# zaiisao/ConTEXTure-NeRF

Hardware: AMD Instinct MI355X
Metric: UNet denoise steps/sec (CFG-batched SD2-depth UNet eval + PLMS update) (higher is better)
Workload: dtype f16; 1 GPU; BASELINE configs[1]: 1 view @768^2 (latent 96^2), 50 PLMS steps (51 UNet evals), SD2-depth UNet fp16, CFG batch 2, guidance 10, random-init weights; mesh substitution napoleon.obj -> n/a for this stage (denoise loop only); latent=96, cfg_batch=2, ctx_len=77, views_per_rank=1, parallelism=view-shard x1

## Files before the change

### contexture-nerf_amd/_lib.py

```python
import ctypes as C
import os
import torch

_HERE = os.path.dirname(os.path.abspath(__file__))
LIB_PATH = os.path.join(_HERE, "libctxnerf.so")

_vp, _i32, _i64, _f32 = C.c_void_p, C.c_int32, C.c_int64, C.c_float

SIGNATURES = {
    "ctx_version": (_i32, []),
    "ctx_last_error": (C.c_char_p, []),
    "ctx_device_check": (_i32, []),
    "ctx_prepare_vertices": (_i32, [_vp, _vp, _vp, _vp, _i32, _i32, _i32, _vp, _vp, _vp, _vp, _vp]),
    "ctx_rasterize_ws_bytes": (_i64, [_i32, _i32, _i32, _i32]),
    "ctx_rasterize_fwd": (_i32, [_i32, _i32, _vp, _vp, _vp, _i32, _i32, _i32, _f32, _f32, _vp, _vp, _vp, _i64, _vp]),
    "ctx_rasterize_fused": (_i32, [_i32, _i32, _vp, _vp, _vp, _i32, _vp, _i32, _i32, _f32, _f32, _vp, _vp, _vp, _vp, _vp, _i64, _vp]),
    "ctx_normalize_depth_ws_bytes": (_i64, [_i32]),
    "ctx_normalize_depth": (_i32, [_vp, _i32, _i32, _vp, _vp, _vp, _vp]),
    "ctx_texture_mapping_fwd": (_i32, [_vp, _vp, _i32, _i32, _i32, _i32, _i32, _i32, _vp, _vp, _vp]),
    "ctx_texture_mapping_bwd": (_i32, [_vp, _vp, _i32, _i32, _i32, _i32, _vp, _vp, _vp]),
    "ctx_texmap_bwd_plan_bytes": (_i64, [_i32, _i32, _i32]),
    "ctx_texmap_bwd_plan": (_i32, [_vp, _vp, _i32, _i32, _i32, _vp, _vp]),
    "ctx_texture_mapping_bwd_binned_ws_bytes": (_i64, [_i32, _i32]),
    "ctx_texture_mapping_bwd_binned": (_i32, [_vp, _vp, _vp, _i32, _i32, _i32, _i32, _vp, _vp, _vp, _vp]),
# ... 109 lines not shown
    "ctx_vae_encode": (_i32, [_vp, _vp, _i32, _i32, _i32, _vp, _vp]),
    "ctx_vae_flops": (C.c_double, [_vp]),
    "ctx_vae_encode_train_workspace_bytes": (_i64, [_vp, _i32, _i32, _i32]),
    "ctx_vae_encode_train": (_i32, [_vp, _vp, _i32, _i32, _i32, _vp, _vp]),
    "ctx_vae_encode_bwd": (_i32, [_vp, _vp, _f32, _vp, _vp]),
    "ctx_gemm_f16": (_i32, [_vp, _vp, _vp, _vp, _i32, _i32, _i32, _vp, _vp]),
    "ctx_conv3x3_f16": (_i32, [_vp, _vp, _vp, _vp, _vp, _i32, _i32, _i32, _i32, _i32, _i32, _i32, _vp, _vp]),
    "ctx_conv3x3_seg_f16": (_i32, [_vp, _vp, _vp, _vp, _vp, _vp, _i32, _i32, _i32, _i32, _i32, _vp, _vp, _i32, _i32, _vp, _vp, _i32, _i32,
                                   _vp, _i32, _vp, _vp]),
    "ctx_conv3x3_gn_f16": (_i32, [_vp, _vp, _vp, _vp, _vp, _vp, _i32, _i32, _i32, _i32, _i32, _vp, _i32, _i32, _i32, _vp, _vp, _vp, _vp]),
    "ctx_gemm_last_kernel": (None, [_vp, _vp]),
    "ctx_conv3x3_geom_f16": (_i32, [_vp, _vp, _vp, _vp, _i32, _i32, _i32, _i32, _i32, _i32, _i32, _i32, _i32, _vp, _i32, _vp, _vp]),
    "ctx_pack_conv3_dgrad_f16": (_i32, [_vp, _i32, _i32, _i32, _vp, _vp]),
    "ctx_pack_conv3_phase_f16": (_i32, [_vp, _i32, _i32, _vp, _vp]),
    "ctx_conv3x3_phase_f16": (_i32, [_vp, _vp, _vp, _vp, _vp, _i32, _i32, _i32, _i32, _i32, _vp, _i32, _vp, _vp]),
    "ctx_pack_mat_dgrad_f16": (_i32, [_vp, _i32, _i32, _i32, _i32, _vp, _vp]),
    "ctx_groupnorm_bwd_ws_bytes": (_i64, [_i32, _i32]),
    "ctx_groupnorm_bwd_f16": (_i32, [_vp, _vp, _vp, _vp, _vp, _i32, _i32, _i32, _i32, _f32, _i32, _vp, _vp, _vp]),
    "ctx_softmax_rows_f16": (_i32, [_vp, _i32, _i32, _f32, _vp, _vp]),
    "ctx_softmax_bwd_rows_f16": (_i32, [_vp, _vp, _i32, _i32, _f32, _vp, _vp]),
    "ctx_quant_bwd_f16": (_i32, [_vp, _vp, _i32, _i32, _i64, _f32, _vp, _vp]),
    "ctx_conv_in_bwd_f16": (_i32, [_vp, _vp, _i32, _i32, _i32, _i32, _i32, _f32, _vp, _vp]),
    "ctx_conv_in_f16": (_i32, [_vp, _vp, _vp, _i32, _i32, _i32, _i32, _i32, _vp, _vp]),
    "ctx_conv_out_f16": (_i32, [_vp, _vp, _vp, _i32, _i32, _i32, _i32, _i32, _vp, _vp]),
    "ctx_gemv_f16": (_i32, [_vp, _vp, _vp, _i32, _i32, _i32, _i32, _i32, _vp, _vp]),
    "ctx_time_embed_f16": (_i32, [_vp, _i32, _i32, _vp, _vp]),
    "ctx_transpose_v_f16": (_i32, [_vp, _i32, _i32, _i32, _i32, _i32, _vp, _vp]),
    "ctx_concat_f16": (_i32, [_vp, _vp, _i64, _i32, _i32, _vp, _vp]),
    "ctx_concat_f32": (_i32, [_vp, _vp, _i64, _i32, _i32, _vp, _vp]),
    "ctx_f32_to_f16": (_i32, [_vp, _i64, _vp, _vp]),
    "ctx_f16_to_f32": (_i32, [_vp, _i64, _vp, _vp]),
    "ctx_conv_small_f16": (_i32, [_vp, _vp, _vp, _vp, _i32, _i32, _i32, _i32, _i32, _i32, _i32, _vp, _vp]),
    "ctx_add_scaled_f16": (_i32, [_vp, _vp, _f32, _i64, _vp]),
    "ctx_pointwise_f32": (_i32, [_vp, _vp, _vp, _i32, _i32, _i64, _i32, _vp, _vp]),
    "ctx_pack_fwd_f16": (_i32, [_vp, _i32, _i32, _i32, _vp, _vp]),
    "ctx_groupnorm_f16": (_i32, [_vp, _vp, _vp, _i32, _i32, _i32, _i32, _f32, _i32, _vp, _vp, _vp]),
    "ctx_groupnorm2_f16": (_i32, [_vp, _vp, _i32, _vp, _vp, _i32, _i32, _i32, _i32, _f32, _i32, _vp, _vp, _vp]),
    "ctx_groupnorm_apply_f16": (_i32, [_vp, _vp, _i32, _vp, _vp, _i32, _i32, _i32, _i32, _f32, _i32, _vp, _vp]),
    "ctx_groupnorm_slabs_f16": (_i32, [_vp, _i32, _vp, _vp, _vp, _i32, _vp, _vp, _i32, _i32, _i32, _i32, _f32, _i32, _vp, _vp]),
    "ctx_layernorm_f16": (_i32, [_vp, _vp, _vp, _i64, _i32, _f32, _vp, _vp]),
    "ctx_attention_ws_bytes": (_i64, [_i32, _i32, _i32]),
    "ctx_attention_f16": (_i32, [_vp, _vp, _vp, _i32, _i32, _i32, _i32, _i32, _i32, _f32, _vp, _i32, _vp, _vp]),
    "ctx_groupnorm_ws_bytes": (_i64, [_i32, _i32]),
    "ctx_geglu_f16": (_i32, [_vp, _i64, _i32, _vp, _vp]),
    "ctx_profile_begin": (_i32, []),
    "ctx_profile_end": (_i32, [_i32, _vp, _vp]),
# ... 61 lines not shown
```

### contexture-nerf_amd/csrc/elementwise.hip

```cpp
#include "common.h"
#include "kernels.h"
#include <math.h>

__global__ __launch_bounds__(256) void k_geglu(const f16 *__restrict__ h, int64_t M, int C4, f16 *__restrict__ y)
{
    const int c8n = C4 / 8;
    const int64_t total = M * c8n;
    for (int64_t i = (int64_t)blockIdx.x * 256 + threadIdx.x; i < total; i += (int64_t)gridDim.x * 256) {
        int64_t m = i / c8n;
        int c8 = (int)(i % c8n);
        f16x8 a = *(const f16x8 *)(h + m * 2 * C4 + c8 * 8);
        f16x8 g = *(const f16x8 *)(h + m * 2 * C4 + C4 + c8 * 8);
        f16x8 o;
#pragma unroll
        for (int j = 0; j < 8; ++j) {
            float gf = (float)g[j];
            o[j] = (f16)((float)a[j] * (0.5f * gf * (1.0f + erff(gf * 0.70710678118654752f))));
        }
        *(f16x8 *)(y + m * C4 + c8 * 8) = o;
    }
}

extern "C" int32_t ctx_geglu_f16(const void *h, int64_t M, int32_t C4, void *y, ctx_stream_t stream)
{
// ... 88 lines not shown
}

__global__ void k_time_embed(const float *__restrict__ t, int B, int dim, f16 *__restrict__ out)
{
    int i = blockIdx.x * blockDim.x + threadIdx.x;
    int half = dim / 2;
    if (i >= half) return;
    float fr = expf(-9.210340371976184f * (float)i / (float)half);
    float a = t[0] * fr;
    float c = cosf(a), sn = sinf(a);
    for (int b = 0; b < B; ++b) {
        out[(size_t)b * dim + i] = (f16)c;
        out[(size_t)b * dim + half + i] = (f16)sn;
    }
}
int ctx_time_embed_core(const float *t, int B, int dim, f16 *out, hipStream_t s)
{
    CTX_REQUIRE(t && out && B > 0 && dim >= 2 && dim % 2 == 0, "time_embed: unsupported B=%d dim=%d", B, dim);
    hipLaunchKernelGGL(k_time_embed, dim3(cdiv(dim / 2, 64)), dim3(64), 0, s, t, B, dim, out);
    CTX_CHECK_LAUNCH("time_embed");
    return CTX_OK;
}

#define CI_SPLIT 16
template <int CP, int CX>
__global__ __launch_bounds__(256) void k_conv_in(const float *__restrict__ x, const f16 *__restrict__ w,
                                                 const f16 *__restrict__ bias, int B, int Cin, int H, int W, int Cout,
                                                 f16 *__restrict__ y)
{
    extern __shared__ __attribute__((aligned(16))) float s_w[];
    constexpr int WR = 9 * CP, WX = 9 * CX;
    const int o8n = Cout / 8;
    const int o8_per = (o8n + CI_SPLIT - 1) / CI_SPLIT;
    const int o8_0 = blockIdx.y * o8_per, o8_1 = min(o8n, o8_0 + o8_per);
    const int no = (o8_1 - o8_0) * 8;
    for (int i = threadIdx.x; i < no * WX; i += 256) {
        const int o = i / WX, r = i - o * WX, t = r / CX, c = r - t * CX;
        s_w[i] = (float)w[(size_t)(o8_0 * 8 + o) * WR + t * CP + c];
    }
    __syncthreads();
    const int64_t npix = (int64_t)B * H * W;
    const int64_t pix0 = (int64_t)blockIdx.x * 256;
    const int64_t pix = pix0 + threadIdx.x;
    const bool live = pix < npix;
    const int64_t pq = live ? pix : npix - 1;
    int b = (int)(pq / (H * W)), p = (int)(pq % (H * W));
    int oy = p / W, ox = p % W;
    float in[9][CX];
#pragma unroll
    for (int t = 0; t < 9; ++t) {
        int iy = oy + t / 3 - 1, ix = ox + t % 3 - 1;
        bool ok = iy >= 0 && iy < H && ix >= 0 && ix < W;
#pragma unroll
        for (int c = 0; c < CX; ++c)
            in[t][c] = (ok && c < Cin) ? (float)(f16)x[(((size_t)b * Cin + c) * H + iy) * W + ix] : 0.f;
    }
    f16 *patch = (f16 *)(s_w + no * WX);
    for (int g0 = o8_0; g0 < o8_1; g0 += 8) {
        const int ng = min(8, o8_1 - g0);
        for (int gi = 0; gi < ng; ++gi) {
            const int o8 = g0 + gi;
            f16x8 o;
#pragma unroll
            for (int j = 0; j < 8; ++j) {
                const float *wr = s_w + ((o8 - o8_0) * 8 + j) * WX;
                float acc = (float)bias[o8 * 8 + j];
#pragma unroll
                for (int t = 0; t < 9; ++t)
#pragma unroll
                    for (int c = 0; c < CX; ++c) acc += in[t][c] * wr[t * CX + c];
                o[j] = (f16)acc;
            }
            *(f16x8 *)(patch + threadIdx.x * 72 + gi * 8) = o;
        }
        __syncthreads();
        for (int ch = threadIdx.x; ch < 256 * ng; ch += 256) {
            const int px = ch / ng, gi = ch - px * ng;
            if (pix0 + px < npix) *(f16x8 *)(y + (pix0 + px) * Cout + (g0 + gi) * 8) = *(const f16x8 *)(patch + px * 72 + gi * 8);
        }
        __syncthreads();
    }
}
int ctx_conv_in_core(const float *x, const f16 *w, const f16 *bias, int B, int Cin, int H, int W, int Cout, f16 *y, hipStream_t s)
{
    CTX_REQUIRE(x && w && bias && y && Cout > 0 && Cout % 8 == 0, "conv_in: unsupported Cout=%d", Cout);
    CTX_REQUIRE(Cin >= 1 && Cin <= 16, "conv_in: need 1 <= Cin <= 16 (Cin=%d)", Cin);
    CTX_REQUIRE(B > 0 && H > 0 && W > 0 && (int64_t)H * W < (1ll << 31), "conv_in: unsupported grid B=%d H=%d W=%d", B, H, W);
    int64_t npix = (int64_t)B * H * W;
    int o8_per = (Cout / 8 + CI_SPLIT - 1) / CI_SPLIT;
    const int cx = Cin <= 3 ? 3 : Cin <= 5 ? Cin : Cin <= 8 ? 8 : Cin == 9 ? 9 : 16;
    CTX_REQUIRE((size_t)o8_per * 8 * 9 * cx * sizeof(float) + 256 * 72 * sizeof(f16) <= 64 * 1024,
                "conv_in: the weight slice of Cout=%d at Cin=%d does not fit the LDS", Cout, Cin);
    const dim3 grid((unsigned)cdiv64(npix, 256), CI_SPLIT);
#define CI_GO(CP_, CX_) hipLaunchKernelGGL((k_conv_in<CP_, CX_>), grid, dim3(256), (size_t)o8_per * 8 * 9 * CX_ * sizeof(float) + 256 * 72 * sizeof(f16), s, x, w, bias, B, Cin, H, W, Cout, y)
    if (Cin <= 3) CI_GO(8, 3);
    else if (Cin == 4) CI_GO(8, 4);
    else if (Cin == 5) CI_GO(8, 5);
    else if (Cin <= 8) CI_GO(8, 8);
    else if (Cin == 9) CI_GO(16, 9);
    else CI_GO(16, 16);
#undef CI_GO
    CTX_CHECK_LAUNCH("conv_in");
    return CTX_OK;
}

template <int NU, bool WF32>
__global__ __launch_bounds__(256) void k_conv_out(const f16 *__restrict__ x, const f16 *__restrict__ w,
                                                  const f16 *__restrict__ bias, int B, int H, int W, int C, int Cout,
                                                  float *__restrict__ out)
{
    extern __shared__ __attribute__((aligned(16))) char s_cw_raw[];
    f16 *s_cw = (f16 *)s_cw_raw;
    float *s_cf = (float *)s_cw_raw;
    const int nwt = Cout * 9 * C;
    if (WF32) {
        for (int i = threadIdx.x * 8; i < nwt; i += 256 * 8) {
            const f16x8 v = *(const f16x8 *)(w + i);
#pragma unroll
            for (int j = 0; j < 8; ++j) s_cf[i + j] = (float)v[j];
        }
    } else {
        for (int i = threadIdx.x * 8; i < nwt; i += 256 * 8) *(f16x8 *)(s_cw + i) = *(const f16x8 *)(w + i);
    }
// ... 135 lines not shown
}
extern "C" int32_t ctx_transpose_v_f16(const void *v, int32_t B, int32_t S, int32_t ld, int32_t heads, int32_t Sp, void *vt, ctx_stream_t stream)
{
    CTX_REQUIRE(B <= 65535 && heads <= 65535, "transpose_v: B=%d / heads=%d exceed the grid", B, heads);
    return ctx_transpose_v_core((const f16 *)v, B, S, ld, heads, Sp, (f16 *)vt, (hipStream_t)stream);
}
extern "C" int32_t ctx_f32_to_f16(const float *x, int64_t n, void *y, ctx_stream_t stream)
{
    return ctx_f32_to_f16_core(x, n, (f16 *)y, (hipStream_t)stream);
}
extern "C" int32_t ctx_f16_to_f32(const void *x, int64_t n, float *y, ctx_stream_t stream)
{
    return ctx_f16_to_f32_core((const f16 *)x, n, y, (hipStream_t)stream);
}
extern "C" int32_t ctx_time_embed_f16(const float *t, int32_t B, int32_t dim, void *out, ctx_stream_t stream)
{
    return ctx_time_embed_core(t, B, dim, (f16 *)out, (hipStream_t)stream);
}
extern "C" int32_t ctx_conv_in_f16(const float *x, const void *w_pack, const void *bias, int32_t B, int32_t Cin, int32_t H, int32_t W, int32_t Cout,
                                   void *y, ctx_stream_t stream)
{
    return ctx_conv_in_core(x, (const f16 *)w_pack, (const f16 *)bias, B, Cin, H, W, Cout, (f16 *)y, (hipStream_t)stream);
}
extern "C" int32_t ctx_conv_out_f16(const void *x, const void *w, const void *bias, int32_t B, int32_t H, int32_t W, int32_t C, int32_t Cout,
                                    float *out, ctx_stream_t stream)
{
    return ctx_conv_out_core((const f16 *)x, (const f16 *)w, (const f16 *)bias, B, H, W, C, Cout, out, (hipStream_t)stream);
}
```

### contexture-nerf_amd/csrc/gemm.hip

```cpp
#include "gemm_common.h"

template <int MI, int NI, bool PH = false>
__device__ __forceinline__ void gemm_epilogue(const GemmArgs &a, f32x16 (&acc)[MI][NI], int mw, int nw, int r, int h, const ConvPhase &ph)
{
#pragma unroll
    for (int mi = 0; mi < MI; ++mi) {
        int m = mw + mi * 32 + r;
        if (m >= ph.M) continue;
        const int mo = PH ? conv_phase_row(a, ph, m) : m;
        int bidx = a.rowbias ? m / a.rows_per_batch : 0;
        if (a.epi == 1) {
            if constexpr (NI == 2) {
                int fbase = nw / 2;
#pragma unroll
                for (int g = 0; g < 4; ++g) {
                    int nn = nw + 8 * g + 4 * h;
                    if (nn >= a.N) continue;
                    f16x4 o;
#pragma unroll
                    for (int j = 0; j < 4; ++j) {
                        float xv = acc[mi][0][4 * g + j], gv = acc[mi][1][4 * g + j];
                        if (a.bias) { xv += (float)a.bias[nn + j]; gv += (float)a.bias[nn + 32 + j]; }
                        o[j] = geglu(xv, gv);
                    }
// ... 666 lines not shown
                                      int32_t B, int32_t H, int32_t W, int32_t Cin, int32_t Cout, void *part, int32_t splitk, int32_t keep_slabs,
                                      int32_t groups, void *gn_part, int32_t *slots, void *y, ctx_stream_t stream)
{
    CTX_REQUIRE(x && w && (y || keep_slabs), "conv3x3_gn: null pointer");
    CTX_REQUIRE(B > 0 && H > 0 && W > 0 && Cin % 64 == 0 && Cout % 8 == 0 && splitk != 0, "conv3x3_gn: need Cin%%64==0, Cout%%8==0 (Cin=%d Cout=%d)", Cin, Cout);
    CTX_REQUIRE(!gn_part || (slots && groups > 0 && Cout % groups == 0 && !keep_slabs), "conv3x3_gn: a partials request needs slots, groups dividing Cout, and no kept slabs");
    CTX_REQUIRE(!keep_slabs || (part && (splitk > 1 || splitk < 0)), "conv3x3_gn: kept slabs need split-K");
    GemmArgs a = {};
    a.Ho = H; a.Wo = W;
    a.X = (const f16 *)x; a.Wt = (const f16 *)w; a.bias = (const f16 *)bias; a.bias2 = (const f16 *)bias2; a.rowbias = (const f16 *)rowbias;
    a.residual = (const f16 *)residual; a.out = (f16 *)y;
    a.M = B * H * W; a.N = Cout; a.K = 9 * Cin; a.ldc = Cout; a.ldr = Cout; a.rows_per_batch = H * W; a.ldrb = Cout;
    a.H = H; a.W = W; a.Cin = Cin; a.stride = 1;
    a.tile = -1; a.use8 = -1;
    if (splitk < 0 && part) ctx_gemm_plan(a, true); else a.splitk = part ? splitk : 1;
    a.part = (float *)part; a.keep_slabs = keep_slabs ? 1 : 0;
    if (gn_part) { a.gn_part = (float *)gn_part; a.gn_cg = Cout / groups; a.gn_hw = H * W; }
    CTX_REQUIRE((int64_t)a.M * Cin < (1ll << 31) && (int64_t)Cout * a.K < (1ll << 31), "conv3x3_gn: tensor too large for 32-bit offsets");
    const int rc = ctx_gemm_dispatch(a, true, (hipStream_t)stream);
    if (slots) *slots = rc != CTX_OK ? 0 : keep_slabs ? a.splitk : a.gn_part ? a.gn_ns : 0;
    return rc;
}

#define GV_U 4
__global__ __launch_bounds__(256) void k_gemv_f16(const f16 *__restrict__ x, const f16 *__restrict__ w,
                                                  const f16 *__restrict__ bias, int Bm, int N, int K, int silu_in,
                                                  int silu_out, f16 *__restrict__ out)
{
    const int lane = threadIdx.x & 63;
    const int n0 = ((blockIdx.x * 256 + threadIdx.x) >> 6) * 2;
    if (n0 >= N) return;
    const int n1 = n0 + 1 < N ? n0 + 1 : n0;
    float acc[2][4] = {{0.f, 0.f, 0.f, 0.f}, {0.f, 0.f, 0.f, 0.f}};
    const f16x8 zero8 = {0, 0, 0, 0, 0, 0, 0, 0};
    for (int k0 = 0; k0 < K; k0 += 512 * GV_U) {
        f16x8 wv[2][GV_U];
#pragma unroll
        for (int u = 0; u < GV_U; ++u) {
            const int k = k0 + u * 512 + lane * 8;
            const int kc = k < K ? k : K - 8;
            wv[0][u] = *(const f16x8 *)(w + (size_t)n0 * K + kc);
            wv[1][u] = *(const f16x8 *)(w + (size_t)n1 * K + kc);
        }
#pragma unroll
        for (int u = 0; u < GV_U; ++u) {
            const int k = k0 + u * 512 + lane * 8;
            if (k >= K) { wv[0][u] = zero8; wv[1][u] = zero8; }
            const int kc = k < K ? k : K - 8;
            for (int b = 0; b < Bm; ++b) {
                f16x8 xv = *(const f16x8 *)(x + (size_t)b * K + kc);
#pragma unroll
                for (int j = 0; j < 8; ++j) {
                    float xf = (float)xv[j];
                    if (silu_in) xf = xf / (1.0f + __expf(-xf));
                    acc[0][b] += xf * (float)wv[0][u][j];
                    acc[1][b] += xf * (float)wv[1][u][j];
                }
            }
        }
    }
    for (int r = 0; r < 2; ++r) {
        const int n = n0 + r;
        for (int b = 0; b < Bm; ++b) {
            float v = wave_sum(acc[r][b]);
            if (lane == 0 && n < N) {
                if (bias) v += (float)bias[n];
                if (silu_out) v = v / (1.0f + __expf(-v));
                out[(size_t)b * N + n] = (f16)v;
            }
        }
    }
}

int ctx_gemv_core(const f16 *x, const f16 *w, const f16 *bias, int Bm, int N, int K, int silu_in, int silu_out, f16 *out,
                 hipStream_t s)
{
    if (!x || !w || !out || Bm < 1 || N < 1 || K % 8 != 0 || K < 8) {
        ctx_set_error("gemv: null pointer, or Bm=%d (>=1) N=%d (>=1) K=%d (%%8)", Bm, N, K);
        return CTX_E_ARG;
    }
    for (int b0 = 0; b0 < Bm; b0 += 4) {
        const int nb = Bm - b0 < 4 ? Bm - b0 : 4;
        hipLaunchKernelGGL(k_gemv_f16, dim3(cdiv(N, 8)), dim3(256), 0, s, x + (size_t)b0 * K, w, bias, nb, N, K, silu_in, silu_out,
                           out + (size_t)b0 * N);
    }
    return CTX_OK;
}
extern "C" int32_t ctx_gemv_f16(const void *x, const void *w, const void *bias, int32_t Bm, int32_t N, int32_t K, int32_t silu_in, int32_t silu_out,
                                void *out, ctx_stream_t stream)
{
    const int rc = ctx_gemv_core((const f16 *)x, (const f16 *)w, (const f16 *)bias, Bm, N, K, silu_in, silu_out, (f16 *)out, (hipStream_t)stream);
    if (rc != CTX_OK) return rc;
    CTX_CHECK_LAUNCH("gemv");
    return CTX_OK;
}

extern "C" float ctx_bench_gemm(const void *A, const void *Wt, const void *bias, const void *residual, int32_t M, int32_t N,
                                int32_t K, void *C, int32_t conv_B, int32_t conv_H, int32_t conv_W, int32_t conv_Cin,
                                int32_t conv_flags, int32_t epi, void *part, int32_t splitk, int32_t iters, ctx_stream_t stream)
{
    hipStream_t s = (hipStream_t)stream;
    GemmArgs a = {};
    a.X = (const f16 *)A; a.Wt = (const f16 *)Wt; a.bias = (const f16 *)bias; a.residual = (const f16 *)residual; a.out = (f16 *)C;
    bool conv = conv_B > 0;
    if (conv) {
        a.stride = (conv_flags & 1) ? 2 : 1; a.ups = (conv_flags & 2) ? 1 : 0;
        int Hv = conv_H << a.ups, Wv = conv_W << a.ups;
// ... 29 lines not shown
```

### contexture-nerf_amd/csrc/kernels.h

```cpp
#pragma once
#include "common.h"

struct GemmArgs {
    const f16 *X;
    const f16 *Wt;
    const f16 *bias;
    const f16 *rowbias;
    const f16 *residual;
    f16 *out;
    int M, N, K;
    int ldc, ldr;
    int rows_per_batch;
    int ldrb;
    int epi;
    int H, W, Cin, Ho, Wo, stride, ups;
    int poff;
    int res32, out32;
    int zins;
    int phase;
    int ntm, ntn;
    int splitk;
    float *part;
    int pk;
    int krot;
// ... 21 lines not shown
}

static inline void ctx_conv3_phase(GemmArgs &a, const f16 *wp)
{
    a.phase = 1; a.Wt = wp; a.K = 4 * a.Cin;
}
static inline int ctx_conv3_phase_ok(int Cin, int Cout, int stride, int ups, int poff, int zins)
{
    return ups == 1 && stride == 1 && poff == 0 && !zins && Cin % 64 == 0 && Cout % 8 == 0;
}
static inline int ctx_conv3_phase_loses(int M, int Cout, int Cin) { return 0; }

int ctx_gemm_dispatch(GemmArgs &a, bool conv, hipStream_t s);
int ctx_gemm8_try(GemmArgs &a, bool conv, bool force, hipStream_t s);
int ctx_conv_halo_try(GemmArgs &a, int ni, hipStream_t s);
int ctx_gemm144_try(GemmArgs &a, bool conv, int form, hipStream_t s);
int ctx_gemm_pick_split(int M, int N, int K, int epi);
void ctx_gemm_plan(GemmArgs &a, bool conv);
int ctx_gemv_core(const f16 *x, const f16 *w, const f16 *bias, int Bm, int N, int K, int silu_in, int silu_out, f16 *out, hipStream_t s);
int ctx_concat_core(const f16 *a, const f16 *b, int64_t M, int Ca, int Cb, f16 *y, hipStream_t s);
int ctx_transpose_v_core(const f16 *v, int B, int S, int ld, int heads, int Sp, f16 *vt, hipStream_t s);
int ctx_f32_to_f16_core(const float *x, int64_t n, f16 *y, hipStream_t s);
int ctx_time_embed_core(const float *t, int B, int dim, f16 *out, hipStream_t s);
int ctx_conv_in_core(const float *x, const f16 *w, const f16 *bias, int B, int Cin, int H, int W, int Cout, f16 *y, hipStream_t s);
int ctx_conv_out_core(const f16 *x, const f16 *w, const f16 *bias, int B, int H, int W, int C, int Cout, float *out, hipStream_t s);
int ctx_attention_core(const f16 *Q, const f16 *K, const f16 *V, int B, int Sq, int Skv, int heads, int q_stride,
                       int kv_stride, float scale, f16 *O, int o_stride, hipStream_t s);
extern "C" int64_t ctx_groupnorm_ws_bytes(int32_t B, int32_t groups);
int ctx_groupnorm_any(const void *x, int x32, const void *gamma, const void *beta, int B, int HW, int C, int groups, float eps, int silu,
                      void *y, void *stats_ws, hipStream_t stream, const void *x2 = nullptr, int Ca = 0);
int ctx_groupnorm_two_pass(int HW, int C, int groups);
int ctx_groupnorm_apply(const void *x, const float *part, int NS, const void *gamma, const void *beta, int B, int HW, int C, int groups, float eps,
                        int silu, void *y, hipStream_t stream);
struct GnSlabs { const float *part; int S; size_t MN; const f16 *bias, *bias2, *rowbias; int ldrb; };
int ctx_groupnorm_slabs(const GnSlabs &sl, const void *gamma, const void *beta, int B, int HW, int C, int groups, float eps, int silu, void *y,
                        hipStream_t stream);
int ctx_layernorm_any(const void *x, int x32, const void *gamma, const void *beta, int64_t rows, int C, float eps, void *y, hipStream_t stream);
int ctx_concat32_core(const float *a, const float *b, int64_t M, int Ca, int Cb, float *y, hipStream_t s);
int ctx_f16_to_f32_core(const f16 *x, int64_t n, float *y, hipStream_t s);
int ctx_conv_small_core(const float *x32, const f16 *x16, const f16 *w, const f16 *bias, int B, int H, int W, int Cin, int Cout, int stride, int silu,
                        f16 *y, hipStream_t s);
int ctx_add_scaled_core(f16 *dst, const f16 *src, float scale, int64_t n, hipStream_t s);
int ctx_pointwise_core(const void *x, const f16 *w, const f16 *b, int B, int C, int64_t HW, bool nhwc16, float *y, hipStream_t s);

bool ctx_prof_on(void);
void ctx_prof_events(int klass, hipEvent_t *a, hipEvent_t *b);
```

### contexture-nerf_amd/csrc/unet.hip

```cpp
#include "engine.h"
#include <string.h>

struct ResP {
    int cin, cout;
    size_t n1g, n1b, c1w, c1b, n2g, n2b, c2w, c2b, scw, scb;
    int temb_row;
};
struct TrP {
    int C, heads;
    size_t ng, nb, piw, pib, l1g, l1b, qkv, o1w, o1b, l2g, l2b, q2, kv2, o2w, o2b, l3g, l3b, f1w, f1b, f2w, f2b, pow_, pob;
    int kv_row;
};
struct LevelP {
    std::vector<ResP> res;
    std::vector<TrP> tr;
    bool has_attn = false, has_sampler = false;
    size_t sw = 0, sb = 0;
    int sc = 0;
};

struct ctx_unet : Engine {
    ctx_unet_config_t cfg;
    size_t ciw, cib, t1w, t1b, t2w, t2b, tpw, tpb, cng, cnb, cow, cob;
    int temb_dim = 0, temb_rows = 0;
// ... 560 lines not shown
    f16 *te1 = u->allocH((size_t)B * u->temb_dim);
    u->note(2, 2.0 * B * ch[0] * u->temb_dim); RUN(ctx_gemv_core(te0, u->W + u->t1w, u->W + u->t1b, B, u->temb_dim, ch[0], 0, 1, te1, u->s));
    f16 *te2 = u->allocH((size_t)B * u->temb_dim);
    u->note(2, 2.0 * B * u->temb_dim * u->temb_dim); RUN(ctx_gemv_core(te1, u->W + u->t2w, u->W + u->t2b, B, u->temb_dim, u->temb_dim, 0, 1, te2, u->s));
    f16 *tproj = u->allocH((size_t)B * u->temb_rows);
    u->note(2, 2.0 * B * u->temb_rows * u->temb_dim); RUN(ctx_gemv_core(te2, u->W + u->tpw, u->W + u->tpb, B, u->temb_rows, u->temb_dim, 0, 0, tproj, u->s));
    f.tproj = tproj;
    f16 *ctx16 = u->allocH((size_t)B * L * c.cross_attention_dim);
    u->note(2, 0); RUN(ctx_f32_to_f16_core(ctx, (int64_t)B * L * c.cross_attention_dim, ctx16, u->s));
    f.ctx16 = ctx16;
    f16 *kv_all = u->allocH((size_t)B * L * u->kv_rows_total);
    op_gemm(u, ctx16, u->kvw, 0, false, nullptr, B * L, u->kv_rows_total, c.cross_attention_dim, kv_all);
    f.kv_all = kv_all;

    int h = H, w = W;
    if (u->res32 && (u->is_controlnet || u->add_res || u->ref_mode)) {
        ctx_set_error("unet: the fp32 residual-stream mode covers the plain UNet forward only");
        return CTX_E_STATE;
    }
    void *x = u->allocS((size_t)B * h * w * ch[0]);
    {
        size_t m0 = u->top;
        f16 *x16 = u->res32 ? u->allocH((size_t)B * h * w * ch[0]) : (f16 *)x;
        u->note(2, 2.0 * B * h * w * ch[0] * c.in_channels * 9); RUN(ctx_conv_in_core(sample, u->W + u->ciw, u->W + u->cib, B, c.in_channels, h, w, ch[0], x16, u->s));
        if (u->res32) { u->note(2, 0); RUN(ctx_f16_to_f32_core(x16, (int64_t)B * h * w * ch[0], (float *)x, u->s)); u->top = m0; }
    }

    auto add_scaled = [&](f16 *dst, const f16 *src, float scale, size_t n) {
        u->note(2, 0);
        RUN(ctx_add_scaled_core(dst, src, scale, (int64_t)n, u->s));
    };
    if (u->is_controlnet) {
        size_t mark = u->top;
        int eh = 8 * H, ew = 8 * W;
        const f16 *cur16 = nullptr;
        const size_t nconv = u->cond_convs.size();
        for (size_t k = 0; k + 1 < nconv; ++k) {
            const ctx_unet::CondConv &cc = u->cond_convs[k];
            int oh = (eh - 1) / cc.stride + 1, ow = (ew - 1) / cc.stride + 1;
            const bool last = k + 2 == nconv;
            f16 *o = (last && u->cn_cache) ? u->cn_cache : u->allocH((size_t)B * oh * ow * cc.cout);
            if (!u->cn_cache_valid) {
                u->note(2, 2.0 * B * oh * ow * cc.cout * cc.cin * 9);
                RUN(ctx_conv_small_core(k == 0 ? u->cn_cond : nullptr, cur16, u->W + cc.w, u->W + cc.b, B, eh, ew, cc.cin, cc.cout, cc.stride, 1, o, u->s));
            }
            cur16 = o; eh = oh; ew = ow;
        }
// ... 267 lines not shown
```

### include/ctx_nerf.h

```cpp
#ifndef CTX_NERF_H
#define CTX_NERF_H
#include <stdint.h>
#ifdef __cplusplus
extern "C" {
#endif

#define CTX_OK 0
#define CTX_E_ARG (-1)
#define CTX_E_LAUNCH (-2)
#define CTX_E_STATE (-3)

typedef void *ctx_stream_t;

int32_t ctx_version(void);
const char *ctx_last_error(void);
int32_t ctx_device_check(void);

int32_t ctx_prepare_vertices(const float *verts, const int64_t *faces, const float *cam,
                             const float *proj3, int32_t B, int32_t V, int32_t F,
                             float *fv_cam, float *fv_img, float *fnorm,
                             void *ws , ctx_stream_t stream);

int64_t ctx_rasterize_ws_bytes(int32_t H, int32_t W, int32_t B, int32_t F);
int32_t ctx_rasterize_fwd(int32_t H, int32_t W, const float *face_z, const float *face_xy,
// ... 271 lines not shown
int32_t ctx_conv3x3_gn_f16(const void *x, const void *w, const void *bias, const void *bias2, const void *rowbias,
                           const void *residual, int32_t B, int32_t H, int32_t W, int32_t Cin, int32_t Cout, void *part,
                           int32_t splitk, int32_t keep_slabs, int32_t groups, void *gn_part, int32_t *slots, void *y,
                           ctx_stream_t stream);
void ctx_gemm_last_kernel(int32_t *tile, int32_t *use8);
int32_t ctx_conv3x3_geom_f16(const void *x, const void *w, const void *bias, const void *residual, int32_t B, int32_t H, int32_t W,
                             int32_t Cin, int32_t Cout, int32_t stride, int32_t upsample, int32_t poff, int32_t zins, void *part,
                             int32_t splitk, void *y, ctx_stream_t stream);
int32_t ctx_pack_conv3_phase_f16(const float *src, int32_t Cout, int32_t Cin, void *dst, ctx_stream_t stream);
int32_t ctx_conv3x3_phase_f16(const void *x, const void *wp, const void *bias, const void *rowbias, const void *residual, int32_t B,
                              int32_t H, int32_t W, int32_t Cin, int32_t Cout, void *part, int32_t splitk, void *y, ctx_stream_t stream);
int32_t ctx_pack_conv3_dgrad_f16(const float *src, int32_t Cout, int32_t Cin, int32_t pad, void *dst, ctx_stream_t stream);
int32_t ctx_pack_mat_dgrad_f16(const float *src, int32_t out, int32_t in, int32_t ld, int32_t col, void *dst, ctx_stream_t stream);
int64_t ctx_groupnorm_bwd_ws_bytes(int32_t B, int32_t groups);
int32_t ctx_groupnorm_bwd_f16(const void *x, const void *dy, const void *gamma, const void *beta, const void *add, int32_t B, int32_t HW,
                              int32_t C, int32_t groups, float eps, int32_t silu, void *dx, void *ws, ctx_stream_t stream);
int32_t ctx_softmax_rows_f16(const void *s, int32_t rows, int32_t n, float scale, void *p, ctx_stream_t stream);
int32_t ctx_softmax_bwd_rows_f16(const void *P, const void *dP, int32_t rows, int32_t n, float scale, void *dS, ctx_stream_t stream);
int32_t ctx_quant_bwd_f16(const float *g, const void *w, int32_t B, int32_t C, int64_t HW, float gscale, void *d, ctx_stream_t stream);
int32_t ctx_conv_in_bwd_f16(const void *dy, const void *w_pack, int32_t B, int32_t H, int32_t W, int32_t C, int32_t Cimg, float inv_gscale,
                            float *dimg, ctx_stream_t stream);
int32_t ctx_conv_in_f16(const float *x, const void *w_pack, const void *bias, int32_t B, int32_t Cin, int32_t H, int32_t W, int32_t Cout,
                        void *y, ctx_stream_t stream);
int32_t ctx_conv_out_f16(const void *x, const void *w, const void *bias, int32_t B, int32_t H, int32_t W, int32_t C, int32_t Cout,
                         float *out, ctx_stream_t stream);
int32_t ctx_gemv_f16(const void *x, const void *w, const void *bias, int32_t Bm, int32_t N, int32_t K, int32_t silu_in, int32_t silu_out,
                     void *out, ctx_stream_t stream);
int32_t ctx_time_embed_f16(const float *t, int32_t B, int32_t dim, void *out, ctx_stream_t stream);
int32_t ctx_transpose_v_f16(const void *v, int32_t B, int32_t S, int32_t ld, int32_t heads, int32_t Sp, void *vt, ctx_stream_t stream);
int32_t ctx_concat_f16(const void *a, const void *b, int64_t M, int32_t Ca, int32_t Cb, void *y, ctx_stream_t stream);
int32_t ctx_concat_f32(const float *a, const float *b, int64_t M, int32_t Ca, int32_t Cb, float *y, ctx_stream_t stream);
int32_t ctx_f32_to_f16(const float *x, int64_t n, void *y, ctx_stream_t stream);
int32_t ctx_f16_to_f32(const void *x, int64_t n, float *y, ctx_stream_t stream);
int32_t ctx_conv_small_f16(const float *x32, const void *x16, const void *w, const void *bias, int32_t B, int32_t H, int32_t W, int32_t Cin,
                           int32_t Cout, int32_t stride, int32_t silu, void *y, ctx_stream_t stream);
int32_t ctx_add_scaled_f16(void *dst, const void *src, float scale, int64_t n, ctx_stream_t stream);
int32_t ctx_pointwise_f32(const void *x, const void *w, const void *b, int32_t B, int32_t C, int64_t HW, int32_t nhwc16, float *y,
                          ctx_stream_t stream);
int32_t ctx_pack_fwd_f16(const float *src, int32_t kind, int32_t a, int32_t b, void *dst, ctx_stream_t stream);
int64_t ctx_groupnorm_ws_bytes(int32_t B, int32_t groups);
int32_t ctx_groupnorm_f16(const void *x, const void *gamma, const void *beta, int32_t B, int32_t HW,
                          int32_t C, int32_t groups, float eps, int32_t silu, void *y, void *stats_ws,
                          ctx_stream_t stream);
int32_t ctx_groupnorm2_f16(const void *xa, const void *xb, int32_t Ca, const void *gamma, const void *beta, int32_t B,
                           int32_t HW, int32_t C, int32_t groups, float eps, int32_t silu, void *y, void *stats_ws,
                           ctx_stream_t stream);
// ... 38 lines not shown
```

Before: 119.4 steps/s.

## Fuse GroupNorm partial stats into conv_in and retile conv_in and gemv kernels

conv_in is restructured so each block handles several pixels per lane over a channel slice, with bias stored in LDS. When the slice aligns with group boundaries, it also writes per-slot GroupNorm partial sums, so the first GroupNorm can skip its own statistics pass over the activation. The gemv kernel is templated on rows per wave and unroll depth chosen from N and K. This adds template variants and more register pressure from the P-pixel input arrays.

Result: no change. 119.6 steps/s (median of 6 runs) (+0.2%).

```diff
diff --git a/contexture-nerf_amd/_lib.py b/contexture-nerf_amd/_lib.py
--- a/contexture-nerf_amd/_lib.py
+++ b/contexture-nerf_amd/_lib.py
@@ -155,6 +155,7 @@
     "ctx_quant_bwd_f16": (_i32, [_vp, _vp, _i32, _i32, _i64, _f32, _vp, _vp]),
     "ctx_conv_in_bwd_f16": (_i32, [_vp, _vp, _i32, _i32, _i32, _i32, _i32, _f32, _vp, _vp]),
     "ctx_conv_in_f16": (_i32, [_vp, _vp, _vp, _i32, _i32, _i32, _i32, _i32, _vp, _vp]),
+    "ctx_conv_in_gn_f16": (_i32, [_vp, _vp, _vp, _i32, _i32, _i32, _i32, _i32, _vp, _i32, _vp, _vp, _vp]),
     "ctx_conv_out_f16": (_i32, [_vp, _vp, _vp, _i32, _i32, _i32, _i32, _i32, _vp, _vp]),
     "ctx_gemv_f16": (_i32, [_vp, _vp, _vp, _i32, _i32, _i32, _i32, _i32, _vp, _vp]),
     "ctx_time_embed_f16": (_i32, [_vp, _i32, _i32, _vp, _vp]),
diff --git a/contexture-nerf_amd/csrc/elementwise.hip b/contexture-nerf_amd/csrc/elementwise.hip
--- a/contexture-nerf_amd/csrc/elementwise.hip
+++ b/contexture-nerf_amd/csrc/elementwise.hip
@@ -134,83 +134,123 @@
     return CTX_OK;
 }
 
-#define CI_SPLIT 16
-template <int CP, int CX>
+#define CI_SL 40
+#define CI_SL_MAX 64
+template <int CP, int CX, int P>
 __global__ __launch_bounds__(256) void k_conv_in(const float *__restrict__ x, const f16 *__restrict__ w,
-                                                 const f16 *__restrict__ bias, int B, int Cin, int H, int W, int Cout,
-                                                 f16 *__restrict__ y)
+                                                 const f16 *__restrict__ bias, int Cin, int H, int W, int Cout, int SL, int NSb,
+                                                 f16 *__restrict__ y, float *__restrict__ gn_part, int cg)
 {
     extern __shared__ __attribute__((aligned(16))) float s_w[];
-    constexpr int WR = 9 * CP, WX = 9 * CX;
-    const int o8n = Cout / 8;
-    const int o8_per = (o8n + CI_SPLIT - 1) / CI_SPLIT;
-    const int o8_0 = blockIdx.y * o8_per, o8_1 = min(o8n, o8_0 + o8_per);
-    const int no = (o8_1 - o8_0) * 8;
-    for (int i = threadIdx.x; i < no * WX; i += 256) {
+    constexpr int WR = 9 * CP, WX = 9 * CX, WXP = (WX + 4) & ~3, PB = 64 * P;
+    const int HW = H * W;
+    const int b = blockIdx.x / NSb, slot = blockIdx.x - b * NSb;
+    const int c0 = blockIdx.y * SL, nc = min(SL, Cout - c0);
+    for (int i = threadIdx.x; i < nc * WX; i += 256) {
         const int o = i / WX, r = i - o * WX, t = r / CX, c = r - t * CX;
-        s_w[i] = (float)w[(size_t)(o8_0 * 8 + o) * WR + t * CP + c];
-    }
+        s_w[o * WXP + r] = (float)w[(size_t)(c0 + o) * WR + t * CP + c];
+    }
+    for (int o = threadIdx.x; o < nc; o += 256) s_w[o * WXP + WX] = (float)bias[c0 + o];
     __syncthreads();
-    const int64_t npix = (int64_t)B * H * W;
-    const int64_t pix0 = (int64_t)blockIdx.x * 256;
-    const int64_t pix = pix0 + threadIdx.x;
-    const bool live = pix < npix;
-    const int64_t pq = live ? pix : npix - 1;
-    int b = (int)(pq / (H * W)), p = (int)(pq % (H * W));
-    int oy = p / W, ox = p % W;
-    float in[9][CX];
-#pragma unroll
-    for (int t = 0; t < 9; ++t) {
-        int iy = oy + t / 3 - 1, ix = ox + t % 3 - 1;
-        bool ok = iy >= 0 && iy < H && ix >= 0 && ix < W;
-#pragma unroll
-        for (int c = 0; c < CX; ++c)
-            in[t][c] = (ok && c < Cin) ? (float)(f16)x[(((size_t)b * Cin + c) * H + iy) * W + ix] : 0.f;
-    }
-    f16 *patch = (f16 *)(s_w + no * WX);
-    for (int g0 = o8_0; g0 < o8_1; g0 += 8) {
-        const int ng = min(8, o8_1 - g0);
-        for (int gi = 0; gi < ng; ++gi) {
-            const int o8 = g0 + gi;
-            f16x8 o;
-#pragma unroll
-            for (int j = 0; j < 8; ++j) {
-                const float *wr = s_w + ((o8 - o8_0) * 8 + j) * WX;
-                float acc = (float)bias[o8 * 8 + j];
-#pragma unroll
-                for (int t = 0; t < 9; ++t)
-#pragma unroll
-                    for (int c = 0; c < CX; ++c) acc += in[t][c] * wr[t * CX + c];
-                o[j] = (f16)acc;
+    const int lane = threadIdx.x & 63, wave = threadIdx.x >> 6;
+    const int cw = SL >> 2;
+    const int j0 = wave * cw, j1 = min(nc, j0 + cw);
+    const int p0 = slot * PB;
+    float in[P][9][CX];
+    bool live[P];
+#pragma unroll
+    for (int i = 0; i < P; ++i) {
+        const int p = p0 + 64 * i + lane;
+        live[i] = p < HW;
+        const int pq = live[i] ? p : HW - 1;
+        const int oy = pq / W, ox = pq - oy * W;
+#pragma unroll
+        for (int t = 0; t < 9; ++t) {
+            const int iy = oy + t / 3 - 1, ix = ox + t % 3 - 1;
+            const bool ok = iy >= 0 && iy < H && ix >= 0 && ix < W;
+            const int off = ok ? iy * W + ix : 0;
+#pragma unroll
+            for (int c = 0; c < CX; ++c) {
+                float v = 0.f;
+                if (c < Cin) v = (float)(f16)(x + ((size_t)b * Cin + c) * HW)[off];
+                in[i][t][c] = ok ? v : 0.f;
             }
-            *(f16x8 *)(patch + threadIdx.x * 72 + gi * 8) = o;
-        }
-        __syncthreads();
-        for (int ch = threadIdx.x; ch < 256 * ng; ch += 256) {
-            const int px = ch / ng, gi = ch - px * ng;
-            if (pix0 + px < npix) *(f16x8 *)(y + (pix0 + px) * Cout + (g0 + gi) * 8) = *(const f16x8 *)(patch + px * 72 + gi * 8);
-        }
-        __syncthreads();
-    }
-}
-int ctx_conv_in_core(const float *x, const f16 *w, const f16 *bias, int B, int Cin, int H, int W, int Cout, f16 *y, hipStream_t s)
+        }
+    }
+    f16 *patch = (f16 *)(s_w + SL * WXP);
+    const int ps = SL + 8;
+    float gs = 0.f, gq = 0.f;
+    int gc = 0;
+    for (int j = j0; j < j1; ++j) {
+        const float *wr = (const float *)__builtin_assume_aligned(s_w + j * WXP, 16);
+        const float bj = wr[WX];
+        float acc[P];
+#pragma unroll
+        for (int i = 0; i < P; ++i) acc[i] = bj;
+#pragma unroll
+        for (int t = 0; t < 9; ++t)
+#pragma unroll
+            for (int c = 0; c < CX; ++c) {
+                const float wv = wr[t * CX + c];
+#pragma unroll
+                for (int i = 0; i < P; ++i) acc[i] = fmaf(in[i][t][c], wv, acc[i]);
+            }
+#pragma unroll
+        for (int i = 0; i < P; ++i) {
+            float a = acc[i];
+            asm volatile("" : "+v"(a));
+            const f16 h = (f16)a;
+            patch[(64 * i + lane) * ps + j] = h;
+            const float f = live[i] ? (float)h : 0.f;
+            gs += f; gq += f * f;
+        }
+        if (gn_part && ++gc == cg) {
+            gc = 0;
+            const float ss = wave_sum_dpp(gs), qq = wave_sum_dpp(gq);
+            if (lane == 0) *(float2 *)(gn_part + (((size_t)b * NSb + slot) * (Cout / cg) + (c0 + j) / cg) * 2) = make_float2(ss, qq);
+            gs = 0.f; gq = 0.f;
+        }
+    }
+    __syncthreads();
+    const int n8 = nc >> 3;
+    for (int ch = threadIdx.x; ch < PB * n8; ch += 256) {
+        const int px = ch / n8, k = ch - px * n8;
+        if (p0 + px < HW) *(f16x8 *)(y + ((size_t)b * HW + p0 + px) * Cout + c0 + k * 8) = *(const f16x8 *)(patch + px * ps + k * 8);
+    }
+}
+int ctx_conv_in_core(const float *x, const f16 *w, const f16 *bias, int B, int Cin, int H, int W, int Cout, f16 *y, hipStream_t s, float *gn_part,
+                     int groups, int *gn_ns)
 {
     CTX_REQUIRE(x && w && bias && y && Cout > 0 && Cout % 8 == 0, "conv_in: unsupported Cout=%d", Cout);
     CTX_REQUIRE(Cin >= 1 && Cin <= 16, "conv_in: need 1 <= Cin <= 16 (Cin=%d)", Cin);
     CTX_REQUIRE(B > 0 && H > 0 && W > 0 && (int64_t)H * W < (1ll << 31), "conv_in: unsupported grid B=%d H=%d W=%d", B, H, W);
-    int64_t npix = (int64_t)B * H * W;
-    int o8_per = (Cout / 8 + CI_SPLIT - 1) / CI_SPLIT;
-    const int cx = Cin <= 3 ? 3 : Cin <= 5 ? Cin : Cin <= 8 ? 8 : Cin == 9 ? 9 : 16;
-    CTX_REQUIRE((size_t)o8_per * 8 * 9 * cx * sizeof(float) + 256 * 72 * sizeof(f16) <= 64 * 1024,
-                "conv_in: the weight slice of Cout=%d at Cin=%d does not fit the LDS", Cout, Cin);
-    const dim3 grid((unsigned)cdiv64(npix, 256), CI_SPLIT);
-#define CI_GO(CP_, CX_) hipLaunchKernelGGL((k_conv_in<CP_, CX_>), grid, dim3(256), (size_t)o8_per * 8 * 9 * CX_ * sizeof(float) + 256 * 72 * sizeof(f16), s, x, w, bias, B, Cin, H, W, Cout, y)
-    if (Cin <= 3) CI_GO(8, 3);
-    else if (Cin == 4) CI_GO(8, 4);
-    else if (Cin == 5) CI_GO(8, 5);
-    else if (Cin <= 8) CI_GO(8, 8);
-    else if (Cin == 9) CI_GO(16, 9);
-    else CI_GO(16, 16);
+    const int P = Cin <= 5 ? 3 : Cin <= 9 ? 2 : 1;
+    const int64_t nsb = cdiv64((int64_t)H * W, 64 * P);
+    CTX_REQUIRE(nsb * B < (1ll << 31), "conv_in: unsupported grid B=%d H=%d W=%d", B, H, W);
+    const int o8n = Cout / 8;
+    int SL = 8 * cdiv(o8n, cdiv(o8n, CI_SL / 8));
+    if (gn_ns) *gn_ns = 0;
+    int cg = 0;
+    if (gn_part && groups > 0 && Cout % groups == 0 && nsb <= CTX_GN_MAX_SLOTS) {
+        const int g4 = 4 * (Cout / groups);
+        int sl = g4;
+        while (sl % 8) sl += g4;
+        if (sl <= CI_SL_MAX) {
+            SL = sl * (CI_SL / sl > 1 ? CI_SL / sl : 1);
+            cg = Cout / groups;
+            if (gn_ns) *gn_ns = (int)nsb;
+        }
+    }
+    if (!cg) gn_part = nullptr;
+    const dim3 grid((unsigned)(nsb * B), cdiv(Cout, SL));
+#define CI_GO(CP_, CX_, P_) hipLaunchKernelGGL((k_conv_in<CP_, CX_, P_>), grid, dim3(256), \
+        (size_t)SL * ((9 * CX_ + 4) & ~3) * sizeof(float) + (size_t)64 * P_ * (SL + 8) * sizeof(f16), s, x, w, bias, Cin, H, W, Cout, SL, (int)nsb, y, gn_part, cg)
+    if (Cin <= 3) CI_GO(8, 3, 3);
+    else if (Cin == 4) CI_GO(8, 4, 3);
+    else if (Cin == 5) CI_GO(8, 5, 3);
+    else if (Cin <= 8) CI_GO(8, 8, 2);
+    else if (Cin == 9) CI_GO(16, 9, 2);
+    else CI_GO(16, 16, 1);
 #undef CI_GO
     CTX_CHECK_LAUNCH("conv_in");
     return CTX_OK;
@@ -392,6 +432,12 @@
 {
     return ctx_conv_in_core(x, (const f16 *)w_pack, (const f16 *)bias, B, Cin, H, W, Cout, (f16 *)y, (hipStream_t)stream);
 }
+extern "C" int32_t ctx_conv_in_gn_f16(const float *x, const void *w_pack, const void *bias, int32_t B, int32_t Cin, int32_t H, int32_t W, int32_t Cout,
+                                      void *y, int32_t groups, void *gn_part, int32_t *slots, ctx_stream_t stream)
+{
+    CTX_REQUIRE(gn_part && slots && groups > 0, "conv_in_gn: null pointer or groups=%d < 1", groups);
+    return ctx_conv_in_core(x, (const f16 *)w_pack, (const f16 *)bias, B, Cin, H, W, Cout, (f16 *)y, (hipStream_t)stream, (float *)gn_part, groups, slots);
+}
 extern "C" int32_t ctx_conv_out_f16(const void *x, const void *w, const void *bias, int32_t B, int32_t H, int32_t W, int32_t C, int32_t Cout,
                                     float *out, ctx_stream_t stream)
 {
diff --git a/contexture-nerf_amd/csrc/gemm.hip b/contexture-nerf_amd/csrc/gemm.hip
--- a/contexture-nerf_amd/csrc/gemm.hip
+++ b/contexture-nerf_amd/csrc/gemm.hip
@@ -712,51 +712,58 @@
     return rc;
 }
 
-#define GV_U 4
+template <int R, int U>
 __global__ __launch_bounds__(256) void k_gemv_f16(const f16 *__restrict__ x, const f16 *__restrict__ w,
                                                   const f16 *__restrict__ bias, int Bm, int N, int K, int silu_in,
                                                   int silu_out, f16 *__restrict__ out)
 {
     const int lane = threadIdx.x & 63;
-    const int n0 = ((blockIdx.x * 256 + threadIdx.x) >> 6) * 2;
+    const int n0 = ((blockIdx.x * 256 + threadIdx.x) >> 6) * R;
     if (n0 >= N) return;
-    const int n1 = n0 + 1 < N ? n0 + 1 : n0;
-    float acc[2][4] = {{0.f, 0.f, 0.f, 0.f}, {0.f, 0.f, 0.f, 0.f}};
+    float acc[R][4];
+#pragma unroll
+    for (int r = 0; r < R; ++r)
+#pragma unroll
+        for (int b = 0; b < 4; ++b) acc[r][b] = 0.f;
     const f16x8 zero8 = {0, 0, 0, 0, 0, 0, 0, 0};
-    for (int k0 = 0; k0 < K; k0 += 512 * GV_U) {
-        f16x8 wv[2][GV_U];
-#pragma unroll
-        for (int u = 0; u < GV_U; ++u) {
+    for (int k0 = 0; k0 < K; k0 += 512 * U) {
+        f16x8 wv[R][U];
+#pragma unroll
+        for (int u = 0; u < U; ++u) {
             const int k = k0 + u * 512 + lane * 8;
             const int kc = k < K ? k : K - 8;
-            wv[0][u] = *(const f16x8 *)(w + (size_t)n0 * K + kc);
-            wv[1][u] = *(const f16x8 *)(w + (size_t)n1 * K + kc);
-        }
-#pragma unroll
-        for (int u = 0; u < GV_U; ++u) {
+#pragma unroll
+            for (int r = 0; r < R; ++r) wv[r][u] = *(const f16x8 *)(w + (size_t)min(n0 + r, N - 1) * K + kc);
+        }
+#pragma unroll
+        for (int u = 0; u < U; ++u) {
             const int k = k0 + u * 512 + lane * 8;
-            if (k >= K) { wv[0][u] = zero8; wv[1][u] = zero8; }
-            const int kc = k < K ? k : K - 8;
+            const bool dead = k >= K;
+            const int kc = dead ? K - 8 : k;
             for (int b = 0; b < Bm; ++b) {
                 f16x8 xv = *(const f16x8 *)(x + (size_t)b * K + kc);
 #pragma unroll
                 for (int j = 0; j < 8; ++j) {
-                    float xf = (float)xv[j];
+                    float xf = dead ? 0.f : (float)xv[j];
                     if (silu_in) xf = xf / (1.0f + __expf(-xf));
-                    acc[0][b] += xf * (float)wv[0][u][j];
-                    acc[1][b] += xf * (float)wv[1][u][j];
+#pragma unroll
+                    for (int r = 0; r < R; ++r) acc[r][b] += xf * (float)wv[r][u][j];
                 }
             }
         }
     }
-    for (int r = 0; r < 2; ++r) {
+#pragma unroll
+    for (int r = 0; r < R; ++r) {
         const int n = n0 + r;
-        for (int b = 0; b < Bm; ++b) {
-            float v = wave_sum(acc[r][b]);
-            if (lane == 0 && n < N) {
-                if (bias) v += (float)bias[n];
-                if (silu_out) v = v / (1.0f + __expf(-v));
-                out[(size_t)b * N + n] = (f16)v;
+#pragma unroll
+        for (int b = 0; b < 4; ++b) {
+            if (b < Bm) {
+                float v = wave_sum(acc[r][b]);
+                if (lane == 0 && n < N) {
+                    if (bias) v += (float)bias[n];
+                    if (silu_out) v = v / (1.0f + __expf(-v));
+                    out[(size_t)b * N + n] = (f16)v;
+                }
             }
         }
     }
@@ -769,10 +776,17 @@
         ctx_set_error("gemv: null pointer, or Bm=%d (>=1) N=%d (>=1) K=%d (%%8)", Bm, N, K);
         return CTX_E_ARG;
     }
+    static const int rows_env = ctx_env_int("CTX_GEMV_ROWS", 0);
+    const int R = rows_env == 2 || rows_env == 4 ? rows_env : (N >= 4 * 8 * 256 ? 4 : 2);
+    const int U = K <= 512 ? 1 : K <= 1024 ? 2 : K <= 1536 ? 3 : 4;
     for (int b0 = 0; b0 < Bm; b0 += 4) {
         const int nb = Bm - b0 < 4 ? Bm - b0 : 4;
-        hipLaunchKernelGGL(k_gemv_f16, dim3(cdiv(N, 8)), dim3(256), 0, s, x + (size_t)b0 * K, w, bias, nb, N, K, silu_in, silu_out,
-                           out + (size_t)b0 * N);
+#define GV_GO(R_, U_) hipLaunchKernelGGL((k_gemv_f16<R_, U_>), dim3(cdiv(N, 4 * R_)), dim3(256), 0, s, x + (size_t)b0 * K, w, bias, nb, N, K, silu_in, silu_out, \
+                                         out + (size_t)b0 * N)
+#define GV_U(R_) do { if (U == 1) GV_GO(R_, 1); else if (U == 2) GV_GO(R_, 2); else if (U == 3) GV_GO(R_, 3); else GV_GO(R_, 4); } while (0)
+        if (R == 4) GV_U(4); else GV_U(2);
+#undef GV_U
+#undef GV_GO
     }
     return CTX_OK;
 }
diff --git a/contexture-nerf_amd/csrc/kernels.h b/contexture-nerf_amd/csrc/kernels.h
--- a/contexture-nerf_amd/csrc/kernels.h
+++ b/contexture-nerf_amd/csrc/kernels.h
@@ -67,7 +67,8 @@
 int ctx_transpose_v_core(const f16 *v, int B, int S, int ld, int heads, int Sp, f16 *vt, hipStream_t s);
 int ctx_f32_to_f16_core(const float *x, int64_t n, f16 *y, hipStream_t s);
 int ctx_time_embed_core(const float *t, int B, int dim, f16 *out, hipStream_t s);
-int ctx_conv_in_core(const float *x, const f16 *w, const f16 *bias, int B, int Cin, int H, int W, int Cout, f16 *y, hipStream_t s);
+int ctx_conv_in_core(const float *x, const f16 *w, const f16 *bias, int B, int Cin, int H, int W, int Cout, f16 *y, hipStream_t s,
+                     float *gn_part = nullptr, int groups = 0, int *gn_ns = nullptr);
 int ctx_conv_out_core(const f16 *x, const f16 *w, const f16 *bias, int B, int H, int W, int C, int Cout, float *out, hipStream_t s);
 int ctx_attention_core(const f16 *Q, const f16 *K, const f16 *V, int B, int Sq, int Skv, int heads, int q_stride,
                        int kv_stride, float scale, f16 *O, int o_stride, hipStream_t s);
diff --git a/contexture-nerf_amd/csrc/unet.hip b/contexture-nerf_amd/csrc/unet.hip
--- a/contexture-nerf_amd/csrc/unet.hip
+++ b/contexture-nerf_amd/csrc/unet.hip
@@ -606,7 +606,12 @@
     {
         size_t m0 = u->top;
         f16 *x16 = u->res32 ? u->allocH((size_t)B * h * w * ch[0]) : (f16 *)x;
-        u->note(2, 2.0 * B * h * w * ch[0] * c.in_channels * 9); RUN(ctx_conv_in_core(sample, u->W + u->ciw, u->W + u->cib, B, c.in_channels, h, w, ch[0], x16, u->s));
+        static const int ci_gn = ctx_env_int("CTX_CONV_IN_GN", 1);
+        const GnReq rq = gn_request(u, f.gn_stats, h * w, ch[0], ci_gn && !u->is_controlnet);
+        int ns = 0;
+        u->note(2, 2.0 * B * h * w * ch[0] * c.in_channels * 9);
+        RUN(ctx_conv_in_core(sample, u->W + u->ciw, u->W + u->cib, B, c.in_channels, h, w, ch[0], x16, u->s, rq.part, rq.groups, &ns));
+        if (u->live() && ns > 0) u->gn_tag = Engine::GnTag{x, B, h * w, ch[0], rq.groups, ns};
         if (u->res32) { u->note(2, 0); RUN(ctx_f16_to_f32_core(x16, (int64_t)B * h * w * ch[0], (float *)x, u->s)); u->top = m0; }
     }
 
diff --git a/include/ctx_nerf.h b/include/ctx_nerf.h
--- a/include/ctx_nerf.h
+++ b/include/ctx_nerf.h
@@ -317,6 +317,8 @@
                             float *dimg, ctx_stream_t stream);
 int32_t ctx_conv_in_f16(const float *x, const void *w_pack, const void *bias, int32_t B, int32_t Cin, int32_t H, int32_t W, int32_t Cout,
                         void *y, ctx_stream_t stream);
+int32_t ctx_conv_in_gn_f16(const float *x, const void *w_pack, const void *bias, int32_t B, int32_t Cin, int32_t H, int32_t W, int32_t Cout,
+                           void *y, int32_t groups, void *gn_part, int32_t *slots, ctx_stream_t stream);
 int32_t ctx_conv_out_f16(const void *x, const void *w, const void *bias, int32_t B, int32_t H, int32_t W, int32_t C, int32_t Cout,
                          float *out, ctx_stream_t stream);
 int32_t ctx_gemv_f16(const void *x, const void *w, const void *bias, int32_t Bm, int32_t N, int32_t K, int32_t silu_in, int32_t silu_out,
```
